# kornelski/cavif-rs

Hardware: AMD Instinct MI355X
Metric: MPix/s encoded at speed=4 q=80, 1080p batch; bit-exact vs CPU oracle (higher is better)
Workload: dtype u16 samples / i32 transform / i64 RD cost

## Files before the change

__graft_entry__.py:

```python
import os
import subprocess
import sys

ROOT = os.path.dirname(os.path.abspath(__file__))
sys.path.insert(0, ROOT)

HIPCC_FLAGS = ['--offload-arch=gfx950', '-O2', '-mllvm', '-sink-insts-to-avoid-spills', '-mllvm', '-inline-threshold=1000', '-mllvm', '-disable-machine-licm', '-mllvm', '-phi-node-folding-threshold=1', '-std=c++17', '-ffp-contract=off', '-fPIC', '-shared', '-Wno-unused-variable']


def _digest(sources, flags):
    import hashlib
    h = hashlib.sha256(' '.join(flags).encode())
    for s in sorted(sources):
        with open(s, 'rb') as fh:
            h.update(os.path.basename(s).encode() + b'\0' + fh.read())
    return h.hexdigest()


def _stale(target, sources):
    if not os.path.exists(target):
        return True
    t = os.path.getmtime(target)
    return any(os.path.getmtime(s) > t for s in sources)


def build(force=False):
    csrc = os.path.join(ROOT, 'cavif_rs_amd', 'csrc')
    out = os.path.join(ROOT, 'cavif_rs_amd', 'libmi_avif.so')
    srcs = [os.path.join(csrc, f) for f in os.listdir(csrc)] + [os.path.join(ROOT, 'include', 'mi_avif.h')]
    stamp, want = out + '.stamp', _digest(srcs, HIPCC_FLAGS)
    have = open(stamp).read().strip() if os.path.exists(stamp) and os.path.exists(out) else ''
    if force or have != want:
        hipcc = 'hipcc' if subprocess.call(['which', 'hipcc'], stdout=subprocess.DEVNULL) == 0 else '/opt/rocm/bin/hipcc'
        subprocess.check_call([hipcc] + HIPCC_FLAGS + ['-o', out, os.path.join(csrc, 'mi_avif.hip'), '-lz'])
        with open(stamp, 'w') as fh:
            fh.write(want + '\n')
    cli_src = os.path.join(ROOT, 'cavif_rs_amd', 'cli', 'cavif_mi.cpp')
    cli = os.path.join(ROOT, 'cavif_rs_amd', 'cavif_mi')
    if force or _stale(cli, [cli_src, out, os.path.join(ROOT, 'include', 'mi_avif.h')]):
        subprocess.check_call(['g++', '-O2', '-std=c++17', '-o', cli, cli_src, '-L' + os.path.join(ROOT, 'cavif_rs_amd'), '-lmi_avif', '-lpthread', '-Wl,-rpath,$ORIGIN'])
    subprocess.check_call(['make', '-s', '-C', os.path.join(ROOT, 'oracle')])
    try:
        from tests import emu
        emu.build(force=force)
    except Exception as e:
        print('warning: tests/emu build failed (%s); the -m "not gpu" emulator tests will fail, the product library is unaffected' % e, file=sys.stderr)
    try:
        from tests.helpers import k4_harness
        k4_harness.build_all(force=force)
    except Exception as e:
        print('warning: tests/kernels harness build failed (%s); tests/test_k4_coder.py will fail, the product library is unaffected' % e, file=sys.stderr)
    try:
        from tests.helpers import filters_harness
        filters_harness.build_all(force=force)
    except Exception as e:
        print('warning: tests/kernels filter harness build failed (%s); tests/test_loopfilter_kernels.py will fail, the product library is unaffected' % e, file=sys.stderr)
    try:
        from tests.helpers import predict_harness
        predict_harness.build_all(force=force)
    except Exception as e:
        print('warning: tests/kernels prediction harness build failed (%s); tests/test_predict_kernels.py will fail, the product library is unaffected' % e, file=sys.stderr)
    import cavif_rs_amd
    cavif_rs_amd.load_library()


def smoke():
    import numpy as np
    import cavif_rs_amd as m
    from cavif_rs_amd.synth import synth_image
    from tests.helpers import oracle
    assert m.device_count() >= 1, 'no HIP device visible'
    img = synth_image(256, 192, index=3)
    enc = m.Encoder().with_quality(80).with_speed(4).with_bit_depth(10)
    got = enc.encode_rgb(img)
    ref, cs, _ = oracle.ravif_encode(img, quality=80, speed=4, depth=10)
    assert got.avif_file[4:12] == b'ftypavif'
    assert got.avif_file == ref, 'HIP path and CPU oracle disagree (%d vs %d bytes)' % (len(got.avif_file), len(ref))
    print('smoke ok: %dx%d -> %d bytes (colour %d), identical to the oracle' % (img.shape[1], img.shape[0], len(got.avif_file), got.color_byte_size))


if __name__ == '__main__':
    build(force='--force' in sys.argv)
    if '--smoke' in sys.argv:
        smoke()
```

cavif_rs_amd/csrc/dev_group.h:

```cpp
#pragma once
#include "dev_predict.h"
#include "dev_txfm.h"
#include "dev_rate.h"

struct GroupBuf8 {
  int32_t tbuf[8 * 9];
  int32_t cbuf[64];
  int32_t qc[64];
  uint16_t rec[64];
  uint8_t lev[144];
};
#define GROUP_LANE (LANE & 15)
#define GROUP_ID (LANE >> 4)

template <int CTRL> __device__ __forceinline__ int dpp_row_(int v) { return __builtin_amdgcn_update_dpp(0, v, CTRL, 0xF, 0xF, false); }
__device__ __forceinline__ int row_sum_i32(int v) { v += dpp_row_<0x128>(v); v += dpp_row_<0x124>(v); v += dpp_row_<0x122>(v); v += dpp_row_<0x121>(v); return v; }
__device__ __forceinline__ int row_max_i32(int v) {
  v = imax_(v, dpp_row_<0x128>(v)); v = imax_(v, dpp_row_<0x124>(v)); v = imax_(v, dpp_row_<0x122>(v)); v = imax_(v, dpp_row_<0x121>(v)); return v;
}

static __device__ const int tx4_tab[2][3][4][8] = {
  { { { 2896, 2896, 2896, 2896, 0, 0, 0, 0 }, { 3784, 1567, -1567, -3784, 0, 0, 0, 0 }, { 2896, -2896, -2896, 2896, 0, 0, 0, 0 }, { 1567, -3784, 3784, -1567, 0, 0, 0, 0 } },
    { { 1321, 2482, 3344, 3803, 0, 0, 0, 0 }, { 3344, 3344, 0, -3344, 0, 0, 0, 0 }, { 3803, -1321, -3344, 2482, 0, 0, 0, 0 }, { 2482, -3803, 3344, -1321, 0, 0, 0, 0 } },
    { { 5793, 0, 0, 0, 0, 0, 0, 0 }, { 0, 5793, 0, 0, 0, 0, 0, 0 }, { 0, 0, 5793, 0, 0, 0, 0, 0 }, { 0, 0, 0, 5793, 0, 0, 0, 0 } } },
  { { { 2896, 0, 2896, 0, 0, 3784, 0, 1567 }, { 2896, 0, -2896, 0, 0, 1567, 0, -3784 }, { 2896, 0, -2896, 0, 0, 1567, 0, -3784 }, { 2896, 0, 2896, 0, 0, 3784, 0, 1567 } },
    { { 1321, 3344, 3803, 2482, 0, 0, 0, 0 }, { 2482, 3344, -1321, -3803, 0, 0, 0, 0 }, { 3344, 0, -3344, 3344, 0, 0, 0, 0 }, { 3803, -3344, 2482, -1321, 0, 0, 0, 0 } },
    { { 5793, 0, 0, 0, 0, 0, 0, 0 }, { 0, 5793, 0, 0, 0, 0, 0, 0 }, { 0, 0, 5793, 0, 0, 0, 0, 0 }, { 0, 0, 0, 5793, 0, 0, 0, 0 } } } };
__device__ __forceinline__ int tx4_dot(int v, const int *m) {
  int acc = __mul24(m[0], dpp_row_<0x00>(v)) + 2048;
  acc += __mul24(m[1], dpp_row_<0x55>(v));
  acc += __mul24(m[2], dpp_row_<0xAA>(v));
  acc += __mul24(m[3], dpp_row_<0xFF>(v));
  return acc >> 12;
}
__device__ __forceinline__ int tx4_fwd(int v, int kind) { return tx4_dot(v, tx4_tab[0][kind][LANE & 3]); }
__device__ __forceinline__ int tx4_inv(int v, int kind) {
  const int *m = tx4_tab[1][kind][LANE & 3];
  const int e = tx4_dot(v, m), o = tx4_dot(v, m + 4);
  return (LANE & 2) ? e - o : e + o;
}
__device__ __forceinline__ int group_transpose4(int v) { return __shfl(v, (LANE & 48) | ((LANE & 3) << 2) | ((LANE >> 2) & 3)); }

struct GroupRes { int eob, cul, dcc, sse; uint32_t rate; };

template <int CTRL> __device__ __forceinline__ int dpp_row_z(int v) { return __builtin_amdgcn_update_dpp(0, v, CTRL, 0xF, 0xF, false); }
template <typename FP>
__device__ __forceinline__ void eval_group4_tail(const CoefCost &cc, FP f, LDS GroupBuf8 *gb, int coef, int t_src, int t_rec, int tidx, int plane, int txs, int txtype, int ck, int rk,
                                                 int skip_ctx, int dc_ctx, int tx_off, uint32_t tx_cost, int psy_sv, int psy_act, GroupRes *res) {
  constexpr int N = 4, nc = 16;
  const int gl = GROUP_LANE, row = gl >> 2, col = gl & 3, bd = f->bd;
  const int dcq = f->dc_q[plane], acq = f->ac_q[plane];
  const uint32_t dc_recip = f->dc_recip[plane], ac_recip = f->ac_recip[plane];
  const int cls = tx_class_of(txtype), pt = plane > 0, txs_ctx = txs;
  const uint32_t dc_off = (uint32_t)(dcq * 109 / 256), off0 = (uint32_t)(acq * 98 / 256), off1 = (uint32_t)(acq * 109 / 256), off_eob = (uint32_t)(acq * 88 / 256);
  const uint32_t thr = (uint32_t)acq - off_eob, uq = (uint32_t)acq;
  const int c = cls == TXC_2D ? lut4(0xFEA9DB83C7426510ULL, gl) : (cls == TXC_VERT ? gl : col * 4 + row);
  const uint32_t mag = (uint32_t)iabs_(coef); const int neg = coef < 0;
  const int last = row_max_i32((c >= 1 && mag >= thr) ? c + 1 : 0);
  int l0 = 0;
  if (gl == 0) {
    const uint32_t x0 = mag + dc_off;
    uint32_t l0u = __umulhi(x0, dc_recip);
    if (x0 - l0u * (uint32_t)dcq >= (uint32_t)dcq) l0u++;
    l0 = (int)l0u;
  }
  l0 = row_max_i32(l0);
  int eob = last;
  if (eob == 0) eob = l0 ? 1 : 0;
  int lv = 0;
  if (c < eob) {
    if (c == 0) lv = l0;
    else {
      uint32_t lv0 = __umulhi(mag, ac_recip);
      if (mag - lv0 * uq >= uq) lv0++;
      const uint32_t off = lv0 > 0 ? off1 : off0;
      lv = (int)lv0 + ((mag + off) >= (lv0 + 1) * uq);
    }
  }
  gb->qc[gl] = neg ? -lv : lv;
  int dq;
  {
    const int dmx = (1 << (7 + bd)) - 1, dmn = -(1 << (7 + bd));
    uint32_t m = (uint32_t)lv * (uint32_t)(gl == 0 ? dcq : acq);
    m &= 0xFFFFFF;
    const int v = neg ? -(int)m : (int)m;
    dq = v < dmn ? dmn : (v > dmx ? dmx : v);
  }
  const int l15 = imin_(lv, 15);
  const int s1 = dpp_row_z<0x101>(l15), s2 = dpp_row_z<0x102>(l15), s3 = dpp_row_z<0x103>(l15), s5 = dpp_row_z<0x105>(l15);
  const int b1 = dpp_row_z<0x104>(l15), b2 = dpp_row_z<0x108>(l15), b3 = dpp_row_z<0x10C>(l15);
  const int r1 = col < 3 ? s1 : 0, r2 = col < 2 ? s2 : 0, r3 = col < 1 ? s3 : 0, d1 = col < 3 ? s5 : 0;
  uint32_t head = cc.txb[(txs_ctx * 13 + skip_ctx) * CDF_TXB_SKIP_STRIDE + (eob == 0)];
  int bits = 0, cul = 0, dcc = 0;
  if (eob > 0) {
    if (tx_off >= 0) head += tx_cost;
    const int eob_pt = eob_to_pt(eob);
    head += cc.eobpt[0][(pt * 2 + (cls == TXC_2D ? 0 : 1)) * CDF_EOB_PT_16_STRIDE + eob_pt - 1];
    if (eob_pt >= 3) {
      const int nb = eob_pt - 2, rem = eob - ((1 << (eob_pt - 2)) + 1), hi = (rem >> (nb - 1)) & 1;
      head += cc.eobx[((txs_ctx * 2 + pt) * 9 + (eob_pt - 3)) * CDF_EOB_EXTRA_STRIDE + hi];
      head += 512u * (uint32_t)(nb - 1);
    }
    if (c < eob) {
      const int level = lv;
      if (c == eob - 1) {
        const int ctx = c == 0 ? 0 : (c <= nc / 8 ? 1 : (c <= nc / 4 ? 2 : 3));
        bits += cc.beob[((txs_ctx * 2 + pt) * 4 + ctx) * CDF_COEFF_BASE_EOB_STRIDE + imin_(level, 3) - 1];
      } else {
        int mag2 = imin_(r1, 3) + imin_(b1, 3), ctx;
        if (cls == TXC_2D) {
          mag2 += imin_(d1, 3) + imin_(r2, 3) + imin_(b2, 3);
          const int m = imin_((mag2 + 1) >> 1, 4);
          ctx = (row == 0 && col == 0) ? 0 : (row + col < 2 ? m + 1 : (row + col < 4 ? m + 6 : m + 21));
        } else if (cls == TXC_VERT) {
          mag2 += imin_(b2, 3) + imin_(b3, 3);
          const int m = imin_((mag2 + 1) >> 1, 4);
          ctx = m + (row == 0 ? 26 : (row == 1 ? 31 : 36));
        } else {
          mag2 += imin_(r2, 3) + imin_(r3, 3);
          const int m = imin_((mag2 + 1) >> 1, 4);
          ctx = m + (col == 0 ? 26 : (col == 1 ? 31 : 36));
        }
        bits += cc.base[((txs_ctx * 2 + pt) * 42 + ctx) * CDF_COEFF_BASE_STRIDE + imin_(level, 3)];
      }
      if (level > 2) {
        int mg = r1 + b1, ctx;
        if (cls == TXC_2D) { mg = imin_((mg + d1 + 1) >> 1, 6); ctx = c == 0 ? mg : ((row < 2 && col < 2) ? mg + 7 : mg + 14); }
        else if (cls == TXC_HORIZ) { mg = imin_((mg + r2 + 1) >> 1, 6); ctx = c == 0 ? mg : (col == 0 ? mg + 7 : mg + 14); }
        else { mg = imin_((mg + b2 + 1) >> 1, 6); ctx = c == 0 ? mg : (row == 0 ? mg + 7 : mg + 14); }
        const int off = ((imin_(txs_ctx, 3) * 2 + pt) * 21 + ctx) * CDF_COEFF_BR_STRIDE;
        int rem = level - 3;
        for (int idx = 0; idx < 4; idx++) { const int s2 = imin_(rem, 3); bits += cc.br[off + s2]; rem -= s2; if (s2 < 3) break; }
      }
      if (level) {
        if (c == 0) { bits += cc.dcs[(pt * 3 + dc_ctx) * CDF_DC_SIGN_STRIDE + neg]; dcc = neg ? 1 : 2; }
        else bits += 512;
        if (level > 14) { const int len = 32 - __clz(level - 14); bits += 512 * (2 * len - 1); }
      }
      cul += level;
    }
  }
  bits = row_sum_i32(bits);
  const int cd = row_sum_i32(imin_(cul, 63) | (dcc << 16));
  res->eob = eob; res->cul = imin_(cd & 0xFFFF, 63); res->dcc = cd >> 16; res->rate = head + (uint32_t)bits;
  if (eob > 0) {
    const int cbits = imax_(bd + 6, 16), cmax = (1 << (cbits - 1)) - 1, cmin = -(1 << (cbits - 1));
    int v = iclamp_(tx4_inv(dq, rk), cmin, cmax);
    v = group_transpose4(v);
    t_rec = iclamp_(t_rec + round2_(tx4_inv(v, ck), 4), 0, (1 << bd) - 1);
  }
  gb->rec[tidx] = (uint16_t)t_rec;
  WAVE_SYNC();
  const int d = t_src - t_rec;
  const int s = row_sum_i32(__mul24(d, d));
  if (psy_sv >= 0) { const int sd = row_sum_i32(t_rec), qd = row_sum_i32(__mul24(t_rec, t_rec)); res->sse = psy_cell_dist((uint32_t)s, (uint32_t)sd, (uint32_t)qd, (uint32_t)psy_sv, (uint32_t)psy_act, 4, bd); }
  else res->sse = (int)(((unsigned long long)(uint32_t)s * (uint32_t)psy_act + 8192) >> 14);
}

template <int N, typename CostPtr>
__device__ inline void eval_group(const CoefCost &cc, CostPtr cost, const LDS uint16_t *ls, const LDS FrameDev *f, LDS GroupBuf8 *gb,
                                  const LDS uint16_t *src, const LDS uint16_t *pred, int plane, int txs, int txtype,
                                  int skip_ctx, int dc_ctx, int tx_off, int tx_sym, int psy_sv, int psy_act, GroupRes *res) {
  constexpr int P = N + 1, nc = N * N, IT = nc / 16, bwl = N == 4 ? 2 : 3, st = N + 4;
  const int gl = GROUP_LANE;
  const int bd = f->bd;
  const uint32_t tx_cost = cost[tx_off >= 0 ? tx_off + tx_sym : 0];
  int ck, rk; tx_kinds(txtype, &ck, &rk);
  [[maybe_unused]] int t_src = 0, t_rec = 0;
  [[maybe_unused]] const int tidx = ((gl & 3) << 2) | (gl >> 2);
  if constexpr (N == 4) {
    t_src = src[tidx]; t_rec = pred[tidx];
    int v = tx4_fwd((int)((uint32_t)(t_src - t_rec) << 2), ck);
    v = group_transpose4(v);
    const int coef = tx4_fwd(v, rk);
    eval_group4_tail(cc, f, gb, coef, t_src, t_rec, tidx, plane, txs, txtype, ck, rk, skip_ctx, dc_ctx, tx_off, tx_cost, psy_sv, psy_act, res);
    return;
  } else {
#pragma unroll
  for (int k = 0; k < IT; k++) {
    const int idx = gl + 16 * k, i = idx / N, j = idx % N;
    const int pv = pred[idx];
    gb->tbuf[i * P + j] = (int)src[idx] - pv;
    gb->rec[idx] = (uint16_t)pv;
  }
  for (int i = gl; i < 36; i += 16) ((LDS uint32_t *)gb->lev)[i] = 0;
  WAVE_SYNC();
  if (gl < N) {
    int32_t x[N];
#pragma unroll
    for (int r = 0; r < N; r++) x[r] = (int32_t)((uint32_t)gb->tbuf[r * P + gl] << 2);
    tx1d<N>(x, ck, true);
#pragma unroll
    for (int r = 0; r < N; r++) gb->tbuf[r * P + gl] = N == 8 ? rshift_round_(x[r], 1) : x[r];
  }
  WAVE_SYNC();
  if (gl < N) {
    int32_t x[N];
#pragma unroll
    for (int c = 0; c < N; c++) x[c] = gb->tbuf[gl * P + c];
    tx1d<N>(x, rk, true);
#pragma unroll
    for (int c = 0; c < N; c++) gb->cbuf[gl * N + c] = x[c];
  }
  WAVE_SYNC();
  }
  const int dcq = f->dc_q[plane], acq = f->ac_q[plane];
  const uint32_t dc_recip = f->dc_recip[plane], ac_recip = f->ac_recip[plane];
  const int cls = tx_class_of(txtype), pt = plane > 0, txs_ctx = txs;
  const uint32_t dc_off = (uint32_t)(dcq * 109 / 256), off0 = (uint32_t)(acq * 98 / 256), off1 = (uint32_t)(acq * 109 / 256), off_eob = (uint32_t)(acq * 88 / 256);
  const uint32_t thr = (uint32_t)acq - off_eob, uq = (uint32_t)acq;
  int pos[IT]; uint32_t mag[IT]; int neg[IT];
  int last = 0;
#pragma unroll
  for (int k = 0; k < IT; k++) {
    const int i = gl + 16 * k;
    pos[k] = scan_pos(ls, N, cls, i);
    const int c = gb->cbuf[pos[k]];
    mag[k] = (uint32_t)iabs_(c); neg[k] = c < 0;
    if (i >= 1 && mag[k] >= thr) last = i + 1;
  }
  last = row_max_i32(last);
  const uint32_t x0 = (uint32_t)iabs_(gb->cbuf[0]) + dc_off;
  uint32_t l0u = __umulhi(x0, dc_recip);
  if (x0 - l0u * (uint32_t)dcq >= (uint32_t)dcq) l0u++;
  const int l0 = (int)l0u;
  int eob = last;
  if (eob == 0) eob = l0 ? 1 : 0;
  const int dmx = (1 << (7 + bd)) - 1, dmn = -(1 << (7 + bd));
  int lvl[IT];
  WAVE_SYNC();
#pragma unroll
  for (int k = 0; k < IT; k++) {
    const int i = gl + 16 * k;
    int lv = 0;
    if (i < eob) {
      if (i == 0) lv = l0;
      else {
        const uint32_t a = mag[k];
        uint32_t lv0 = __umulhi(a, ac_recip);
        if (a - lv0 * uq >= uq) lv0++;
        const uint32_t off = lv0 > 0 ? off1 : off0;
        lv = (int)lv0 + ((a + off) >= (lv0 + 1) * uq);
      }
    }
    lvl[k] = lv;
    const int pp = pos[k];
    gb->qc[pp] = neg[k] ? -lv : lv;
    gb->lev[(pp >> bwl) * st + (pp & (N - 1))] = (uint8_t)imin_(lv, 127);
    uint32_t m = (uint32_t)lv * (uint32_t)(pp == 0 ? dcq : acq);
    m &= 0xFFFFFF;
    const int v = neg[k] ? -(int)m : (int)m;
    gb->cbuf[pp] = v < dmn ? dmn : (v > dmx ? dmx : v);
  }
  WAVE_SYNC();
  uint32_t head = cc.txb[(txs_ctx * 13 + skip_ctx) * CDF_TXB_SKIP_STRIDE + (eob == 0)];
  int bits = 0, cul = 0, dcc = 0;
  if (eob > 0) {
    if (tx_off >= 0) head += tx_cost;
    const int eob_pt = eob_to_pt(eob);
    head += cc.eobpt[N == 4 ? 0 : 1][(pt * 2 + (cls == TXC_2D ? 0 : 1)) * (N == 4 ? CDF_EOB_PT_16_STRIDE : CDF_EOB_PT_64_STRIDE) + eob_pt - 1];
    if (eob_pt >= 3) {
      const int nb = eob_pt - 2, rem = eob - ((1 << (eob_pt - 2)) + 1), hi = (rem >> (nb - 1)) & 1;
      head += cc.eobx[((txs_ctx * 2 + pt) * 9 + (eob_pt - 3)) * CDF_EOB_EXTRA_STRIDE + hi];
      head += 512u * (uint32_t)(nb - 1);
    }
#pragma unroll
    for (int k = 0; k < IT; k++) {
      const int c = gl + 16 * k;
      if (c < eob) {
        const int pp = pos[k], row = pp >> bwl, col = pp & (N - 1), level = lvl[k];
        const LDS uint8_t *L = gb->lev + row * st + col;
        if (c == eob - 1) {
          const int ctx = c == 0 ? 0 : (c <= nc / 8 ? 1 : (c <= nc / 4 ? 2 : 3));
          bits += cc.beob[((txs_ctx * 2 + pt) * 4 + ctx) * CDF_COEFF_BASE_EOB_STRIDE + imin_(level, 3) - 1];
        } else {
          const int ctx = base_ctx(L, st, cls, row, col);
          bits += cc.base[((txs_ctx * 2 + pt) * 42 + ctx) * CDF_COEFF_BASE_STRIDE + imin_(level, 3)];
        }
        if (level > 2) {
          const int ctx = br_ctx(L, st, cls, row, col, c);
          const int off = ((imin_(txs_ctx, 3) * 2 + pt) * 21 + ctx) * CDF_COEFF_BR_STRIDE;
          int rem = level - 3;
          for (int idx = 0; idx < 4; idx++) { const int s2 = imin_(rem, 3); bits += cc.br[off + s2]; rem -= s2; if (s2 < 3) break; }
        }
        if (level) {
          if (c == 0) { bits += cc.dcs[(pt * 3 + dc_ctx) * CDF_DC_SIGN_STRIDE + neg[k]]; dcc = neg[k] ? 1 : 2; }
          else bits += 512;
          if (level > 14) { const int len = 32 - __clz(level - 14); bits += 512 * (2 * len - 1); }
        }
        cul += level;
      }
    }
  }
  bits = row_sum_i32(bits);
  const int cd = row_sum_i32(imin_(cul, 63) | (dcc << 16));
  res->eob = eob; res->cul = imin_(cd & 0xFFFF, 63); res->dcc = cd >> 16; res->rate = head + (uint32_t)bits;
  {
    constexpr int ROWSH = N == 4 ? 0 : 1;
    const int cbits = imax_(bd + 6, 16), cmax = (1 << (cbits - 1)) - 1, cmin = -(1 << (cbits - 1));
    if constexpr (N == 4) {
      if (eob > 0) {
        int v = iclamp_(tx4_inv(gb->cbuf[gl], rk), cmin, cmax);
        v = group_transpose4(v);
        t_rec = iclamp_(t_rec + round2_(tx4_inv(v, ck), 4), 0, (1 << bd) - 1);
        gb->rec[tidx] = (uint16_t)t_rec;
      }
      WAVE_SYNC();
    } else {
      const bool act = gl < N && eob > 0;
      if (act) {
        int32_t x[N];
  #pragma unroll
        for (int j = 0; j < N; j++) x[j] = gb->cbuf[gl * N + j];
        tx1d<N>(x, rk, false);
  #pragma unroll
        for (int j = 0; j < N; j++) gb->tbuf[gl * P + j] = iclamp_(round2_(x[j], ROWSH), cmin, cmax);
      }
      WAVE_SYNC();
      const int mx = (1 << bd) - 1;
      if (act) {
        int32_t x[N];
  #pragma unroll
        for (int i = 0; i < N; i++) x[i] = gb->tbuf[i * P + gl];
        tx1d<N>(x, ck, false);
  #pragma unroll
        for (int i = 0; i < N; i++) gb->rec[i * N + gl] = (uint16_t)iclamp_((int)gb->rec[i * N + gl] + round2_(x[i], 4), 0, mx);
      }
      WAVE_SYNC();
    }
  }
  int s = 0, sd = 0, qd = 0;
  if constexpr (N == 4) { const int d = t_src - t_rec; s = __mul24(d, d); sd = t_rec; qd = __mul24(t_rec, t_rec); }
  else
#pragma unroll
  for (int k = 0; k < IT; k++) { const int idx = gl + 16 * k; const int rv = gb->rec[idx], d = (int)src[idx] - rv; s += __mul24(d, d); sd += rv; qd += __mul24(rv, rv); }
  s = row_sum_i32(s);
  if (psy_sv >= 0) { sd = row_sum_i32(sd); qd = row_sum_i32(qd); res->sse = psy_cell_dist((uint32_t)s, (uint32_t)sd, (uint32_t)qd, (uint32_t)psy_sv, (uint32_t)psy_act, N == 4 ? 4 : 8, bd); }
  else res->sse = (int)(((unsigned long long)(uint32_t)s * (uint32_t)psy_act + 8192) >> 14);
}

struct GroupPredBuf { uint16_t wa[48], wl[48], tmp[32], pred[64]; };

__device__ __forceinline__ void edge_filter_group(LDS uint16_t *buf, int sz, int strength, LDS uint16_t *tmp, int gl) {
  if (strength) for (int i = gl; i < sz; i += 16) tmp[i] = buf[i - 1];
  WAVE_SYNC();
  if (strength) for (int i = 1 + gl; i < sz; i += 16) {
    int s = 0;
#pragma unroll
    for (int j = 0; j < 5; j++) {
      const int k = iclamp_(i - 2 + j, 0, sz - 1);
      const int kw = strength == 1 ? (j == 0 || j == 4 ? 0 : (j == 2 ? 8 : 4)) : (strength == 2 ? (j == 0 || j == 4 ? 0 : (j == 2 ? 6 : 5)) : (j == 0 || j == 4 ? 2 : 4));
      s += kw * tmp[k];
    }
    buf[i - 1] = (uint16_t)((s + 8) >> 4);
  }
  WAVE_SYNC();
}
__device__ __forceinline__ void edge_upsample_group(LDS uint16_t *buf, int num_px, int on, int bd, LDS uint16_t *tmp, int gl) {
  if (on) for (int i = gl; i < num_px + 3; i += 16) {
    uint16_t v;
    if (i == 0) v = buf[-1]; else if (i == num_px + 2) v = buf[num_px - 1]; else v = buf[i - 2];
    tmp[i] = v;
  }
  WAVE_SYNC();
  const int mx = (1 << bd) - 1;
  if (on) {
    if (gl == 0) buf[-2] = tmp[0];
    for (int i = gl; i < num_px; i += 16) {
      int s = -(int)tmp[i] + 9 * (int)tmp[i + 1] + 9 * (int)tmp[i + 2] - (int)tmp[i + 3];
      s = iclamp_(round2_(s, 4), 0, mx);
      buf[2 * i - 1] = (uint16_t)s;
      buf[2 * i] = tmp[i + 2];
    }
  }
  WAVE_SYNC();
}

template <int N>
__device__ inline void predict_dir_group(const LDS FrameDev *f, int x, int y, int have_left, int have_above, int pa, int ftype,
                                         const LDS uint16_t *ra, const LDS uint16_t *rl, LDS GroupPredBuf *gp, LDS uint16_t *out = nullptr) {
  constexpr int log2w = N == 4 ? 2 : 3, nn = N * N;
  const int gl = GROUP_LANE, bd = f->bd;
  const int max_x = f->mi_cols * 4 - 1, max_y = f->mi_rows * 4 - 1;
  LDS uint16_t *wa = gp->wa + EDGE_OFF, *wl = gp->wl + EDGE_OFF;
  for (int i = gl; i < 2 * N + 1; i += 16) { wa[i - 1] = ra[i - 1]; wl[i - 1] = rl[i - 1]; }
  WAVE_SYNC();
  const int diag = pa != 90 && pa != 180;
  {
    const int st_a = (diag && have_above) ? edge_strength_dev(N, N, ftype, pa - 90) : 0;
    const int num_a = imin_(N, max_x - x + 1) + (pa < 90 ? N : 0) + 1;
    edge_filter_group(wa, num_a, st_a, gp->tmp, gl);
    const int st_l = (diag && have_left) ? edge_strength_dev(N, N, ftype, pa - 180) : 0;
    const int num_l = imin_(N, max_y - y + 1) + (pa > 180 ? N : 0) + 1;
    edge_filter_group(wl, num_l, st_l, gp->tmp, gl);
  }
  const int up_a = edge_upsample_sel_dev(N, N, ftype, pa - 90);
  edge_upsample_group(wa, N + (pa < 90 ? N : 0), up_a, bd, gp->tmp, gl);
  const int up_l = edge_upsample_sel_dev(N, N, ftype, pa - 180);
  edge_upsample_group(wl, N + (pa > 180 ? N : 0), up_l, bd, gp->tmp, gl);
  int dx = 0, dy = 0;
  if (pa < 90) dx = dr_deriv_dev(pa); else if (pa > 90 && pa < 180) dx = dr_deriv_dev(180 - pa);
  if (pa > 90 && pa < 180) dy = dr_deriv_dev(pa - 90); else if (pa > 180) dy = dr_deriv_dev(270 - pa);
  for (int idx = gl; idx < nn; idx += 16) {
    const int i = idx >> log2w, j = idx & (N - 1);
    int v;
    if (pa < 90) {
      const int max_base = (2 * N - 1) << up_a;
      const int id = (i + 1) * dx, base = (id >> (6 - up_a)) + (j << up_a), sh = ((id << up_a) >> 1) & 0x1F;
      v = base < max_base ? round2_(wa[base] * (32 - sh) + wa[base + 1] * sh, 5) : wa[max_base];
    } else if (pa > 90 && pa < 180) {
      int id = (j << 6) - (i + 1) * dx, base = id >> (6 - up_a);
      if (base >= -(1 << up_a)) { const int sh = ((id << up_a) >> 1) & 0x1F; v = round2_(wa[base] * (32 - sh) + wa[base + 1] * sh, 5); }
      else { id = (i << 6) - (j + 1) * dy; base = id >> (6 - up_l); const int sh = ((id << up_l) >> 1) & 0x1F; v = round2_(wl[base] * (32 - sh) + wl[base + 1] * sh, 5); }
    } else if (pa > 180) {
      const int id = (j + 1) * dy, base = (id >> (6 - up_l)) + (i << up_l), sh = ((id << up_l) >> 1) & 0x1F;
      v = round2_(wl[base] * (32 - sh) + wl[base + 1] * sh, 5);
    } else if (pa == 90) v = wa[j];
    else v = wl[i];
    (out ? out : (LDS uint16_t *)gp->pred)[idx] = (uint16_t)v;
  }
  WAVE_SYNC();
}

template <int N>
__device__ inline void predict_nondir_group(int mode, int have_left, int have_above, int bd, const LDS uint16_t *ra, const LDS uint16_t *rl, LDS uint16_t *pred) {
  constexpr int log2w = N == 4 ? 2 : 3, IT = N * N / 16;
  constexpr unsigned long long wt = N == 4 ? 0x405595FFULL : 0x202532496992C5FFULL;
  const int gl = GROUP_LANE;
  if (mode == DC_PRED) {
    int v = 1 << (bd - 1);
    if (have_left || have_above) {
      int s = gl < N ? (have_above ? (int)ra[gl] : 0) + (have_left ? (int)rl[gl] : 0) : 0;
      s = row_sum_i32(s);
      v = (have_left && have_above) ? (s + N) >> (log2w + 1) : (s + (N >> 1)) >> log2w;
    }
#pragma unroll
    for (int k = 0; k < IT; k++) pred[gl + 16 * k] = (uint16_t)v;
  } else if (mode == PAETH_PRED) {
    const int tl = ra[-1];
#pragma unroll
    for (int k = 0; k < IT; k++) {
      const int idx = gl + 16 * k, i = idx >> log2w, j = idx & (N - 1);
      const int a = ra[j], l = rl[i], base = a + l - tl;
      const int pl = iabs_(base - l), pt = iabs_(base - a), ptl = iabs_(base - tl);
      pred[idx] = (uint16_t)((pl <= pt && pl <= ptl) ? l : (pt <= ptl ? a : tl));
    }
  } else if (mode >= 0) {
    const int bl = rl[N - 1], tr = ra[N - 1];
#pragma unroll
    for (int k = 0; k < IT; k++) {
      const int idx = gl + 16 * k, i = idx >> log2w, j = idx & (N - 1);
      const int wi = lut8(wt, i), wj = lut8(wt, j);
      const int vt = wi * (int)ra[j] + (256 - wi) * bl, ht = wj * (int)rl[i] + (256 - wj) * tr;
      pred[idx] = (uint16_t)(mode == SMOOTH_PRED ? round2_(vt + ht, 9) : round2_(mode == SMOOTH_V_PRED ? vt : ht, 8));
    }
  }
  WAVE_SYNC();
}

__device__ __forceinline__ int satd8_lane(int d0, int d1, int d2, int d3);
template <int N> __device__ inline int satd_group(const LDS uint16_t *src, const LDS uint16_t *pred) {
  constexpr int units = N * (N / 4);
  const int u = GROUP_LANE;
  if constexpr (N == 8) {
    const int xx = (u & 3) + ((u >> 1) & 4), o = (u & 4) * N + xx;
    const int d0 = (int)src[o] - (int)pred[o], d1 = (int)src[o + N] - (int)pred[o + N];
    const int d2 = (int)src[o + 2 * N] - (int)pred[o + 2 * N], d3 = (int)src[o + 3 * N] - (int)pred[o + 3 * N];
    return (row_sum_i32(satd8_lane(d0, d1, d2, d3)) + 2) >> 2;
  }
  int s = 0;
  if (u < units) {
    const int xx = u % N, o = (u / N) * 4 * N + xx;
    const int d0 = (int)src[o] - (int)pred[o], d1 = (int)src[o + N] - (int)pred[o + N];
    const int d2 = (int)src[o + 2 * N] - (int)pred[o + 2 * N], d3 = (int)src[o + 3 * N] - (int)pred[o + 3 * N];
    const int a = d0 + d1, b = d0 - d1, c = d2 + d3, e = d2 - d3;
    int t[4] = { a + c, b + e, a - c, b - e };
#pragma unroll
    for (int i = 0; i < 4; i++) {
      int v = __builtin_amdgcn_update_dpp(0, t[i], 0xB1, 0xF, 0xF, false);
      v = (LANE & 1) ? v - t[i] : t[i] + v;
      int w2 = __builtin_amdgcn_update_dpp(0, v, 0x4E, 0xF, 0xF, false);
      v = (LANE & 2) ? w2 - v : v + w2;
      s += iabs_(v);
    }
  }
  return row_sum_i32(s);
}
```

cavif_rs_amd/csrc/dev_predict.h:

```cpp
#pragma once
#include "dev_common.h"

#define EDGE_OFF 16
#define EDGE_LEN(N) (EDGE_OFF + 2 * (N) + 16)

__device__ __forceinline__ const uint8_t *sm_weights_dev(int log2w) {
  static __device__ const uint8_t w4[4] = { 255, 149, 85, 64 };
  static __device__ const uint8_t w8[8] = { 255, 197, 146, 105, 73, 50, 37, 32 };
  static __device__ const uint8_t w16[16] = { 255, 225, 196, 170, 145, 123, 102, 84, 68, 54, 43, 33, 26, 20, 17, 16 };
  static __device__ const uint8_t w32[32] = { 255, 240, 225, 210, 196, 182, 169, 157, 145, 133, 122, 111, 101, 92, 83, 74,
                                              66, 59, 52, 45, 39, 34, 29, 25, 21, 17, 14, 12, 10, 9, 8, 8 };
  static __device__ const uint8_t w64[64] = { 255, 248, 240, 233, 225, 218, 210, 203, 196, 189, 182, 176, 169, 163, 156, 150,
                                              144, 138, 133, 127, 121, 116, 111, 106, 101, 96, 91, 86, 82, 77, 73, 69,
                                              65, 61, 57, 54, 50, 47, 44, 41, 38, 35, 32, 29, 27, 25, 22, 20,
                                              18, 16, 15, 13, 12, 10, 9, 8, 7, 6, 6, 5, 5, 4, 4, 4 };
  switch (log2w) { case 2: return w4; case 3: return w8; case 4: return w16; case 5: return w32; default: return w64; }
}
__device__ __forceinline__ int dr_deriv_dev(int a) {
  switch (a) {
    case 3: return 1023; case 6: return 547; case 9: return 372; case 14: return 273; case 17: return 215;
    case 20: return 178; case 23: return 151; case 26: return 132; case 29: return 116; case 32: return 102;
    case 36: return 90; case 39: return 80; case 42: return 71; case 45: return 64; case 48: return 57;
    case 51: return 51; case 54: return 45; case 58: return 40; case 61: return 35; case 64: return 31;
    case 67: return 27; case 70: return 23; case 73: return 19; case 76: return 15; case 81: return 11;
    case 84: return 7; case 87: return 3; default: return 0;
  }
}
__device__ __forceinline__ int edge_strength_dev(int w, int h, int ft, int delta) {
  const int d = iabs_(delta), blk = w + h; int s = 0;
  if (ft == 0) {
    if (blk <= 8) { if (d >= 56) s = 1; }
    else if (blk <= 12) { if (d >= 40) s = 1; }
    else if (blk <= 16) { if (d >= 40) s = 1; }
    else if (blk <= 24) { if (d >= 8) s = 1; if (d >= 16) s = 2; if (d >= 32) s = 3; }
    else if (blk <= 32) { if (d >= 1) s = 1; if (d >= 4) s = 2; if (d >= 32) s = 3; }
    else { if (d >= 1) s = 3; }
  } else {
    if (blk <= 8) { if (d >= 40) s = 1; if (d >= 64) s = 2; }
    else if (blk <= 16) { if (d >= 20) s = 1; if (d >= 48) s = 2; }
    else if (blk <= 24) { if (d >= 4) s = 3; }
    else { if (d >= 1) s = 3; }
  }
  return s;
}
__device__ __forceinline__ int edge_upsample_sel_dev(int w, int h, int ft, int delta) {
  const int d = iabs_(delta), blk = w + h;
  if (d <= 0 || d >= 40) return 0;
  return ft == 0 ? (blk <= 16) : (blk <= 8);
}

__device__ inline void load_edges(const LDS FrameDev *f, int plane, int x, int y, int n, int have_left, int have_above,
                                  int have_ar, int have_bl, LDS uint16_t *above , LDS uint16_t *left) {
  const int bd = f->bd, rs = f->stride;
  const uint16_t *rec = f->rec[plane];
  const int max_x = f->mi_cols * 4 - 1, max_y = f->mi_rows * 4 - 1;
  const int tot = 2 * n;
  const int na = x + (have_ar ? 2 * n : n) - 1, nl = y + (have_bl ? 2 * n : n) - 1;
  const int lim_a = imin_(max_x, na), lim_l = imin_(max_y, nl);
  for (int i = LANE; i <= tot; i += 64) {
    const bool corner = i == tot;
    int ia, il;
    if (have_above) ia = (y - 1) * rs + (corner ? (have_left ? x - 1 : x) : imin_(lim_a, x + i));
    else ia = y * rs + (have_left ? x - 1 : x);
    if (have_left) il = imin_(lim_l, y + i) * rs + x - 1;
    else il = (have_above ? y - 1 : y) * rs + x;
    uint16_t a = rec[ia], l = rec[il];
    if (!have_above && !have_left) { a = (uint16_t)(corner ? (1 << (bd - 1)) : (1 << (bd - 1)) - 1); l = (uint16_t)((1 << (bd - 1)) + 1); }
    if (corner) { above[-1] = a; left[-1] = a; }
    else { above[i] = a; left[i] = l; }
  }
  WAVE_SYNC();
}

__device__ inline void edge_filter_dev(LDS uint16_t *buf, int sz, int strength, LDS uint16_t *tmp) {
  if (!strength) return;
  for (int i = LANE; i < sz; i += 64) tmp[i] = buf[i - 1];
  WAVE_SYNC();
  for (int i = 1 + LANE; i < sz; i += 64) {
    int s = 0;
#pragma unroll
    for (int j = 0; j < 5; j++) {
      const int k = iclamp_(i - 2 + j, 0, sz - 1);
      const int kw = strength == 1 ? (j == 0 || j == 4 ? 0 : (j == 2 ? 8 : 4)) : (strength == 2 ? (j == 0 || j == 4 ? 0 : (j == 2 ? 6 : 5)) : (j == 0 || j == 4 ? 2 : 4));
      s += kw * tmp[k];
    }
    buf[i - 1] = (uint16_t)((s + 8) >> 4);
  }
  WAVE_SYNC();
}
__device__ inline void edge_upsample_dev(LDS uint16_t *buf, int num_px, int bd, LDS uint16_t *tmp) {
  for (int i = LANE; i < num_px + 3; i += 64) {
    uint16_t v;
    if (i == 0) v = buf[-1]; else if (i == num_px + 2) v = buf[num_px - 1]; else v = buf[i - 2];
    tmp[i] = v;
  }
  WAVE_SYNC();
  const int mx = (1 << bd) - 1;
  if (LANE == 0) buf[-2] = tmp[0];
  for (int i = LANE; i < num_px; i += 64) {
    int s = -(int)tmp[i] + 9 * (int)tmp[i + 1] + 9 * (int)tmp[i + 2] - (int)tmp[i + 3];
    s = iclamp_(round2_(s, 4), 0, mx);
    buf[2 * i - 1] = (uint16_t)s;
    buf[2 * i] = tmp[i + 2];
  }
  WAVE_SYNC();
}

__device__ inline void predict_block(const LDS FrameDev *f, int x, int y, int log2w, int have_left, int have_above,
                                     int mode, int angle_delta, int ftype, const LDS uint16_t *ra, const LDS uint16_t *rl,
                                     LDS uint16_t *wa, LDS uint16_t *wl, LDS uint16_t *tmp, LDS uint16_t *pred) {
  const int n = 1 << log2w, bd = f->bd, nn = n * n;
  const int max_x = f->mi_cols * 4 - 1, max_y = f->mi_rows * 4 - 1;
  if (mode == PAETH_PRED) {
    const int tl = ra[-1];
    for (int idx = LANE; idx < nn; idx += 64) {
      const int i = idx >> log2w, j = idx & (n - 1);
      const int base = ra[j] + rl[i] - tl;
      const int pl = iabs_(base - rl[i]), pt = iabs_(base - ra[j]), ptl = iabs_(base - tl);
      pred[idx] = (pl <= pt && pl <= ptl) ? rl[i] : (pt <= ptl ? ra[j] : (uint16_t)tl);
    }
  } else if (mode == DC_PRED) {
    int v;
    if (have_left || have_above) {
      int s = 0;
      for (int k = LANE; k < n; k += 64) s += (have_above ? ra[k] : 0) + (have_left ? rl[k] : 0);
      s = wave_sum_i32(s);
      if (have_left && have_above) v = (s + n) / (2 * n);
      else v = (s + (n >> 1)) >> log2w;
    } else v = 1 << (bd - 1);
    for (int idx = LANE; idx < nn; idx += 64) pred[idx] = (uint16_t)v;
  } else if (mode == SMOOTH_PRED || mode == SMOOTH_V_PRED || mode == SMOOTH_H_PRED) {
    const uint8_t *sw = sm_weights_dev(log2w);
    const int bl = rl[n - 1], tr = ra[n - 1];
    for (int idx = LANE; idx < nn; idx += 64) {
      const int i = idx >> log2w, j = idx & (n - 1);
      int p;
      if (mode == SMOOTH_PRED) p = round2_(sw[i] * ra[j] + (256 - sw[i]) * bl + sw[j] * rl[i] + (256 - sw[j]) * tr, 9);
      else if (mode == SMOOTH_V_PRED) p = round2_(sw[i] * ra[j] + (256 - sw[i]) * bl, 8);
      else p = round2_(sw[j] * rl[i] + (256 - sw[j]) * tr, 8);
      pred[idx] = (uint16_t)p;
    }
  } else {
    const int pa = mode_angle_of(mode) + angle_delta * 3;
    for (int i = LANE; i < 2 * n + 1; i += 64) { wa[i - 1] = ra[i - 1]; wl[i - 1] = rl[i - 1]; }
    WAVE_SYNC();
    int up_a = 0, up_l = 0;
    if (pa != 90 && pa != 180) {
      if (pa > 90 && pa < 180 && 2 * n >= 24) {
        if (LANE == 0) { const int v = round2_(wl[0] * 5 + wa[-1] * 6 + wa[0] * 5, 4); wa[-1] = (uint16_t)v; wl[-1] = (uint16_t)v; }
        WAVE_SYNC();
      }
      if (have_above) {
        const int st = edge_strength_dev(n, n, ftype, pa - 90);
        const int num = imin_(n, max_x - x + 1) + (pa < 90 ? n : 0) + 1;
        edge_filter_dev(wa, num, st, tmp);
      }
      if (have_left) {
        const int st = edge_strength_dev(n, n, ftype, pa - 180);
        const int num = imin_(n, max_y - y + 1) + (pa > 180 ? n : 0) + 1;
        edge_filter_dev(wl, num, st, tmp);
      }
    }
    up_a = edge_upsample_sel_dev(n, n, ftype, pa - 90);
    if (up_a) edge_upsample_dev(wa, n + (pa < 90 ? n : 0), bd, tmp);
    up_l = edge_upsample_sel_dev(n, n, ftype, pa - 180);
    if (up_l) edge_upsample_dev(wl, n + (pa > 180 ? n : 0), bd, tmp);
    int dx = 0, dy = 0;
    if (pa < 90) dx = dr_deriv_dev(pa); else if (pa > 90 && pa < 180) dx = dr_deriv_dev(180 - pa);
    if (pa > 90 && pa < 180) dy = dr_deriv_dev(pa - 90); else if (pa > 180) dy = dr_deriv_dev(270 - pa);
    for (int idx = LANE; idx < nn; idx += 64) {
      const int i = idx >> log2w, j = idx & (n - 1);
      int v;
      if (pa < 90) {
        const int max_base = (2 * n - 1) << up_a;
        const int id = (i + 1) * dx, base = (id >> (6 - up_a)) + (j << up_a), sh = ((id << up_a) >> 1) & 0x1F;
        v = base < max_base ? round2_(wa[base] * (32 - sh) + wa[base + 1] * sh, 5) : wa[max_base];
      } else if (pa > 90 && pa < 180) {
        int id = (j << 6) - (i + 1) * dx, base = id >> (6 - up_a);
        if (base >= -(1 << up_a)) { const int sh = ((id << up_a) >> 1) & 0x1F; v = round2_(wa[base] * (32 - sh) + wa[base + 1] * sh, 5); }
        else { id = (i << 6) - (j + 1) * dy; base = id >> (6 - up_l); const int sh = ((id << up_l) >> 1) & 0x1F; v = round2_(wl[base] * (32 - sh) + wl[base + 1] * sh, 5); }
      } else if (pa > 180) {
        const int id = (j + 1) * dy, base = (id >> (6 - up_l)) + (i << up_l), sh = ((id << up_l) >> 1) & 0x1F;
        v = round2_(wl[base] * (32 - sh) + wl[base + 1] * sh, 5);
      } else if (pa == 90) v = wa[j];
      else v = wl[i];
      pred[idx] = (uint16_t)v;
    }
  }
  WAVE_SYNC();
}

__device__ inline void predict_cfl_dev(const LDS FrameDev *f, int x, int y, int log2w, int alpha, const LDS uint16_t *dcp, LDS uint16_t *out) {
  const int n = 1 << log2w, nn = n * n, mx = (1 << f->bd) - 1, rs = f->stride;
  const uint16_t *luma = f->rec[0] + y * rs + x;
  int s = 0;
  for (int idx = LANE; idx < nn; idx += 64) s += luma[(idx >> log2w) * rs + (idx & (n - 1))] << 3;
  s = wave_sum_i32(s);
  const int avg = round2_(s, 2 * log2w);
  for (int idx = LANE; idx < nn; idx += 64) {
    const int l = (luma[(idx >> log2w) * rs + (idx & (n - 1))] << 3) - avg;
    const int v = alpha * l;
    const int sc = v >= 0 ? round2_(v, 6) : -round2_(-v, 6);
    out[idx] = (uint16_t)iclamp_(dcp[idx] + sc, 0, mx);
  }
  WAVE_SYNC();
}
```

Before: 541.8.

## Rewrite directional edge prep with DPP lane shuffles and branchless prediction

Replaces the multi-pass LDS edge filter and upsample steps in group directional prediction with a single register-level pass. Neighbours are exchanged through DPP row shifts, which removes several wave syncs and LDS round trips. The per-pixel directional interpolation becomes branchless, with gathers issued before the arithmetic, and the derivative switch becomes bit-packed table arithmetic. The new lane-shuffle edge handling carries a bit-exactness risk for boundary and upsample cases, and it also adds a row-predictor test harness to the build.

```diff
diff --git a/__graft_entry__.py b/__graft_entry__.py
--- a/__graft_entry__.py
+++ b/__graft_entry__.py
@@ -60,6 +60,11 @@
         predict_harness.build_all(force=force)
     except Exception as e:
         print('warning: tests/kernels prediction harness build failed (%s); tests/test_predict_kernels.py will fail, the product library is unaffected' % e, file=sys.stderr)
+    try:
+        from tests.helpers import rowpred_harness
+        rowpred_harness.build_all(force=force)
+    except Exception as e:
+        print('warning: tests/kernels row predictor harness build failed (%s); tests/test_rowform_predict.py will fail, the product library is unaffected' % e, file=sys.stderr)
     import cavif_rs_amd
     cavif_rs_amd.load_library()
 
diff --git a/cavif_rs_amd/csrc/dev_group.h b/cavif_rs_amd/csrc/dev_group.h
--- a/cavif_rs_amd/csrc/dev_group.h
+++ b/cavif_rs_amd/csrc/dev_group.h
@@ -341,84 +341,64 @@
 
 struct GroupPredBuf { uint16_t wa[48], wl[48], tmp[32], pred[64]; };
 
-__device__ __forceinline__ void edge_filter_group(LDS uint16_t *buf, int sz, int strength, LDS uint16_t *tmp, int gl) {
-  if (strength) for (int i = gl; i < sz; i += 16) tmp[i] = buf[i - 1];
-  WAVE_SYNC();
-  if (strength) for (int i = 1 + gl; i < sz; i += 16) {
-    int s = 0;
-#pragma unroll
-    for (int j = 0; j < 5; j++) {
-      const int k = iclamp_(i - 2 + j, 0, sz - 1);
-      const int kw = strength == 1 ? (j == 0 || j == 4 ? 0 : (j == 2 ? 8 : 4)) : (strength == 2 ? (j == 0 || j == 4 ? 0 : (j == 2 ? 6 : 5)) : (j == 0 || j == 4 ? 2 : 4));
-      s += kw * tmp[k];
-    }
-    buf[i - 1] = (uint16_t)((s + 8) >> 4);
-  }
-  WAVE_SYNC();
-}
-__device__ __forceinline__ void edge_upsample_group(LDS uint16_t *buf, int num_px, int on, int bd, LDS uint16_t *tmp, int gl) {
-  if (on) for (int i = gl; i < num_px + 3; i += 16) {
-    uint16_t v;
-    if (i == 0) v = buf[-1]; else if (i == num_px + 2) v = buf[num_px - 1]; else v = buf[i - 2];
-    tmp[i] = v;
-  }
-  WAVE_SYNC();
-  const int mx = (1 << bd) - 1;
-  if (on) {
-    if (gl == 0) buf[-2] = tmp[0];
-    for (int i = gl; i < num_px; i += 16) {
-      int s = -(int)tmp[i] + 9 * (int)tmp[i + 1] + 9 * (int)tmp[i + 2] - (int)tmp[i + 3];
-      s = iclamp_(round2_(s, 4), 0, mx);
-      buf[2 * i - 1] = (uint16_t)s;
-      buf[2 * i] = tmp[i + 2];
-    }
-  }
-  WAVE_SYNC();
+__device__ __forceinline__ void edge_prepare_group(int v, int corner, int sz, int strength, int up, int num_px, int mx, LDS uint16_t *w, int gl) {
+  const int ws = strength ? strength + 3 : 0, wt = gl < sz - 1 ? ws : 0;
+  const int below = __builtin_amdgcn_update_dpp(corner, v, 0x111, 0xF, 0xF, false);
+  const int above = __builtin_amdgcn_update_dpp(v, v, 0x101, 0xF, 0xF, false);
+  const int fv = (__mul24(wt, below + (gl < sz - 2 ? above : v)) + __mul24(16 - 2 * wt, v) + 8) >> 4;
+  const int m1 = __builtin_amdgcn_update_dpp(corner, fv, 0x111, 0xF, 0xF, false), m2 = __builtin_amdgcn_update_dpp(corner, fv, 0x112, 0xF, 0xF, false);
+  const int p1 = __builtin_amdgcn_update_dpp(fv, fv, 0x101, 0xF, 0xF, false);
+  const int odd = imax_(0, imin_(mx, (9 * (m1 + fv) - m2 - (gl < num_px - 1 ? p1 : fv) + 8) >> 4));
+  const int e = up ? 2 * gl : gl;
+  const bool first = (up != 0) & (gl == 0);
+  w[e] = (uint16_t)fv;
+  w[e - 1] = (uint16_t)(up ? odd : m1);
+  w[first ? -2 : e] = (uint16_t)(first ? corner : fv);
+}
+template <int N> __device__ __forceinline__ int edge_strength_group(int ftype, int delta) {
+  const int d = iabs_(delta), t1 = ftype ? (N == 4 ? 40 : 20) : (N == 4 ? 56 : 40), t2 = ftype ? (N == 4 ? 64 : 48) : 1 << 30;
+  return (int)(d >= t1) + (int)(d >= t2);
+}
+template <int N> __device__ __forceinline__ int edge_upsample_group(int ftype, int delta) {
+  const int d = iabs_(delta);
+  return (int)(d > 0) & (int)(d < 40) & (int)((ftype == 0) | (N == 4));
 }
 
 template <int N>
 __device__ inline void predict_dir_group(const LDS FrameDev *f, int x, int y, int have_left, int have_above, int pa, int ftype,
                                          const LDS uint16_t *ra, const LDS uint16_t *rl, LDS GroupPredBuf *gp, LDS uint16_t *out = nullptr) {
-  constexpr int log2w = N == 4 ? 2 : 3, nn = N * N;
-  const int gl = GROUP_LANE, bd = f->bd;
+  constexpr int log2w = N == 4 ? 2 : 3, IT = N * N / 16;
+  const int gl = GROUP_LANE, mx = (1 << f->bd) - 1;
   const int max_x = f->mi_cols * 4 - 1, max_y = f->mi_rows * 4 - 1;
   LDS uint16_t *wa = gp->wa + EDGE_OFF, *wl = gp->wl + EDGE_OFF;
-  for (int i = gl; i < 2 * N + 1; i += 16) { wa[i - 1] = ra[i - 1]; wl[i - 1] = rl[i - 1]; }
-  WAVE_SYNC();
-  const int diag = pa != 90 && pa != 180;
-  {
-    const int st_a = (diag && have_above) ? edge_strength_dev(N, N, ftype, pa - 90) : 0;
-    const int num_a = imin_(N, max_x - x + 1) + (pa < 90 ? N : 0) + 1;
-    edge_filter_group(wa, num_a, st_a, gp->tmp, gl);
-    const int st_l = (diag && have_left) ? edge_strength_dev(N, N, ftype, pa - 180) : 0;
-    const int num_l = imin_(N, max_y - y + 1) + (pa > 180 ? N : 0) + 1;
-    edge_filter_group(wl, num_l, st_l, gp->tmp, gl);
-  }
-  const int up_a = edge_upsample_sel_dev(N, N, ftype, pa - 90);
-  edge_upsample_group(wa, N + (pa < 90 ? N : 0), up_a, bd, gp->tmp, gl);
-  const int up_l = edge_upsample_sel_dev(N, N, ftype, pa - 180);
-  edge_upsample_group(wl, N + (pa > 180 ? N : 0), up_l, bd, gp->tmp, gl);
-  int dx = 0, dy = 0;
-  if (pa < 90) dx = dr_deriv_dev(pa); else if (pa > 90 && pa < 180) dx = dr_deriv_dev(180 - pa);
-  if (pa > 90 && pa < 180) dy = dr_deriv_dev(pa - 90); else if (pa > 180) dy = dr_deriv_dev(270 - pa);
-  for (int idx = gl; idx < nn; idx += 16) {
-    const int i = idx >> log2w, j = idx & (N - 1);
-    int v;
-    if (pa < 90) {
-      const int max_base = (2 * N - 1) << up_a;
-      const int id = (i + 1) * dx, base = (id >> (6 - up_a)) + (j << up_a), sh = ((id << up_a) >> 1) & 0x1F;
-      v = base < max_base ? round2_(wa[base] * (32 - sh) + wa[base + 1] * sh, 5) : wa[max_base];
-    } else if (pa > 90 && pa < 180) {
-      int id = (j << 6) - (i + 1) * dx, base = id >> (6 - up_a);
-      if (base >= -(1 << up_a)) { const int sh = ((id << up_a) >> 1) & 0x1F; v = round2_(wa[base] * (32 - sh) + wa[base + 1] * sh, 5); }
-      else { id = (i << 6) - (j + 1) * dy; base = id >> (6 - up_l); const int sh = ((id << up_l) >> 1) & 0x1F; v = round2_(wl[base] * (32 - sh) + wl[base + 1] * sh, 5); }
-    } else if (pa > 180) {
-      const int id = (j + 1) * dy, base = (id >> (6 - up_l)) + (i << up_l), sh = ((id << up_l) >> 1) & 0x1F;
-      v = round2_(wl[base] * (32 - sh) + wl[base + 1] * sh, 5);
-    } else if (pa == 90) v = wa[j];
-    else v = wl[i];
-    (out ? out : (LDS uint16_t *)gp->pred)[idx] = (uint16_t)v;
-  }
+  const int k = imin_(gl, 2 * N - 1);
+  const int va = ra[k], vl = rl[k], ca = ra[-1], cl = rl[-1];
+  const bool diag = (pa != 90) & (pa != 180);
+  const int s_a = edge_strength_group<N>(ftype, pa - 90), s_l = edge_strength_group<N>(ftype, pa - 180);
+  const int st_a = (diag & (have_above != 0)) ? s_a : 0, st_l = (diag & (have_left != 0)) ? s_l : 0;
+  const int up_a = edge_upsample_group<N>(ftype, pa - 90), up_l = edge_upsample_group<N>(ftype, pa - 180);
+  edge_prepare_group(va, ca, imin_(N, max_x - x + 1) + (pa < 90 ? N : 0) + 1, st_a, up_a, N + (pa < 90 ? N : 0), mx, wa, gl);
+  edge_prepare_group(vl, cl, imin_(N, max_y - y + 1) + (pa > 180 ? N : 0) + 1, st_l, up_l, N + (pa > 180 ? N : 0), mx, wl, gl);
+  WAVE_SYNC();
+  const int dx = dr_deriv_dev(pa < 90 ? pa : 180 - pa), dy = dr_deriv_dev(pa > 180 ? 270 - pa : pa - 90);
+  const int sdx = pa < 90 ? dx : -dx, sdy = pa > 180 ? dy : -dy;
+  const int max_base = (2 * N - 1) << up_a, switch_base = -(1 << up_a);
+  LDS uint16_t *dst = out ? out : (LDS uint16_t *)gp->pred;
+  int p0[IT], p1[IT], sh[IT];
+#pragma unroll
+  for (int it = 0; it < IT; it++) {
+    const int idx = gl + 16 * it, i = idx >> log2w, j = idx & (N - 1);
+    const int ta = sdx * (i + 1), tl = sdy * (j + 1);
+    const int ba = (j << up_a) + (ta >> (6 - up_a)), bl = (i << up_l) + (tl >> (6 - up_l));
+    const bool over = ba >= max_base, left = (pa >= 180) | (ba < switch_base);
+    const LDS uint16_t *e = left ? wl : wa;
+    const int b_a = over ? max_base : ba, sh_a = over ? 0 : ((ta << up_a) >> 1) & 0x1F;
+    const int b = left ? bl : b_a;
+    sh[it] = left ? ((tl << up_l) >> 1) & 0x1F : sh_a;
+    p0[it] = e[b]; p1[it] = e[b + 1];
+  }
+#pragma unroll
+  for (int it = 0; it < IT; it++) dst[gl + 16 * it] = (uint16_t)round2_(p0[it] * (32 - sh[it]) + p1[it] * sh[it], 5);
   WAVE_SYNC();
 }
 
diff --git a/cavif_rs_amd/csrc/dev_predict.h b/cavif_rs_amd/csrc/dev_predict.h
--- a/cavif_rs_amd/csrc/dev_predict.h
+++ b/cavif_rs_amd/csrc/dev_predict.h
@@ -17,14 +17,17 @@
   switch (log2w) { case 2: return w4; case 3: return w8; case 4: return w16; case 5: return w32; default: return w64; }
 }
 __device__ __forceinline__ int dr_deriv_dev(int a) {
-  switch (a) {
-    case 3: return 1023; case 6: return 547; case 9: return 372; case 14: return 273; case 17: return 215;
-    case 20: return 178; case 23: return 151; case 26: return 132; case 29: return 116; case 32: return 102;
-    case 36: return 90; case 39: return 80; case 42: return 71; case 45: return 64; case 48: return 57;
-    case 51: return 51; case 54: return 45; case 58: return 40; case 61: return 35; case 64: return 31;
-    case 67: return 27; case 70: return 23; case 73: return 19; case 76: return 15; case 81: return 11;
-    case 84: return 7; case 87: return 3; default: return 0;
-  }
+  const unsigned ua = (unsigned)a < 90u ? (unsigned)a : 0u;
+  const unsigned k = (ua * 171u) >> 9, r = ua - 3u * k;
+  const bool hit = (unsigned)((0xf035554000eaaa03ULL >> (2 * k)) & 3) == r;
+  const unsigned long long w01 = k < 8 ? 0x97b2d70000000000ULL : 0x4047505a00667484ULL, w23 = k < 24 ? 0x171b1f23282d3339ULL : 0x000003070b000f13ULL;
+  const unsigned long long w = k < 16 ? w01 : w23;
+  int v = lut8(w, (int)(k & 7));
+  v = k == 1 ? 1023 : v;
+  v = k == 2 ? 547 : v;
+  v = k == 3 ? 372 : v;
+  v = k == 4 ? 273 : v;
+  return hit ? v : 0;
 }
 __device__ __forceinline__ int edge_strength_dev(int w, int h, int ft, int delta) {
   const int d = iabs_(delta), blk = w + h; int s = 0;
```

New measurement: 573.1 (median of 5 runs). +5.8%, better.
